# talmolab/VNL-Brax-Imitation

Hardware: NVIDIA B200
Metric: rodent imitation env-steps/s (higher is better)
Workload: dtype f32

## Files before the change

include/vnl_b200.h:

```cpp
#ifndef VNL_B200_H_
#define VNL_B200_H_

#include <stddef.h>
#include <stdint.h>

#ifdef __cplusplus
extern "C" {
#endif

#define VNL_MAGIC_MODEL 0x4d4c4e56u
#define VNL_MAGIC_TASK 0x544c4e56u
#define VNL_BLOB_VERSION 7
#define VNL_TABLE_OFF 64
#define VNL_MAX_FIELDS 96
#define VNL_DATA_OFF (VNL_TABLE_OFF + 2 * VNL_MAX_FIELDS)

enum VnlModelHdr {
  VNL_MH_NQ = 4, VNL_MH_NV, VNL_MH_NU, VNL_MH_NA, VNL_MH_NBODY, VNL_MH_NJNT, VNL_MH_NGEOM,
  VNL_MH_NPAIR,
  VNL_MH_NCON,
  VNL_MH_NLIMIT,
  VNL_MH_NEFC,
  VNL_MH_SOLVER,
  VNL_MH_ITERATIONS, VNL_MH_LS_ITERATIONS,
  VNL_MH_EULERDAMP,
  VNL_MH_NM,
  VNL_MH_NLEVEL,
  VNL_MH_MAXDEPTH,
  VNL_MH_NROOT,
  VNL_MH_NDSLOT,
  VNL_MH_ENV_WARPS,
  VNL_MH_NASLOT,
  VNL_MH_TA,
  VNL_MH_TD,
  VNL_MH_TIMESTEP = 32, VNL_MH_GRAVITY_X, VNL_MH_GRAVITY_Y, VNL_MH_GRAVITY_Z,
  VNL_MH_TOLERANCE, VNL_MH_LS_TOLERANCE, VNL_MH_IMPRATIO, VNL_MH_MEANINERTIA
};

enum VnlModelField {
  VNL_F_BODY_PARENTID = 0,
  VNL_F_BODY_ROOTID,
  VNL_F_BODY_JNTADR,
  VNL_F_BODY_JNTNUM,
  VNL_F_BODY_DOFADR,
  VNL_F_BODY_DOFNUM,
  VNL_F_BODY_POS,
  VNL_F_BODY_QUAT,
  VNL_F_BODY_IPOS,
  VNL_F_BODY_IQUAT,
  VNL_F_BODY_MASS,
  VNL_F_BODY_INERTIA,
  VNL_F_BODY_INVWEIGHT0,
  VNL_F_JNT_TYPE,
  VNL_F_JNT_QPOSADR,
  VNL_F_JNT_DOFADR,
  VNL_F_JNT_BODYID,
  VNL_F_JNT_LIMITED,
  VNL_F_JNT_POS,
  VNL_F_JNT_AXIS,
  VNL_F_JNT_STIFFNESS,
  VNL_F_JNT_RANGE,
  VNL_F_JNT_MARGIN,
  VNL_F_JNT_SOLREF,
  VNL_F_JNT_SOLIMP,
  VNL_F_DOF_BODYID,
// ... 23 lines not shown
  VNL_F_PAIR_GEOM2,
  VNL_F_PAIR_TYPE,
  VNL_F_PAIR_FRICTION,
  VNL_F_PAIR_SOLREF,
  VNL_F_PAIR_SOLIMP,
  VNL_F_PAIR_INCLUDEMARGIN,
  VNL_F_LEVEL_START,
  VNL_F_LEVEL_BODY,
  VNL_F_DOF_MADR,
  VNL_F_M_COL,
  VNL_F_DOF_DEPTH,
  VNL_F_BODY_SUBTREE_END,
  VNL_F_LIMIT_JNT,
  VNL_F_CON_PAIR,
  VNL_F_CON_SIGN,
  VNL_F_GEOMC_BODY,
  VNL_F_GEOMC_POS,
  VNL_F_GEOMC_MAT,
  VNL_F_PLANE_POS,
  VNL_F_PLANE_MAT,
  VNL_F_BODY_IMAT,
  VNL_F_M_ROW,
  VNL_F_BODY_LASTDOF,
  VNL_F_DESC_ADR,
  VNL_F_DESC_ENTRY,
  VNL_F_DOFLEVEL_START,
  VNL_F_DOFLEVEL_DOF,
  VNL_F_DOF_ACTADR,
  VNL_F_DOF_ACTLIST,
  VNL_F_KTAB,
  VNL_F_MODEL_COUNT
};

enum VnlKtab {
  VNL_KT_LVL_START = 0,
  VNL_KT_LVL_BP,
  VNL_KT_PARENT,
  VNL_KT_CHILD_ADR,
  VNL_KT_CHILD_LIST,
  VNL_KT_BODY_DOFADR,
  VNL_KT_BODY_DOFNUM,
  VNL_KT_BODY_TREE,
  VNL_KT_BODY_LASTDOF,
  VNL_KT_SUB_END,
  VNL_KT_ROOTS,
  VNL_KT_MROW,
  VNL_KT_MCOL,
  VNL_KT_DOF_BODY,
  VNL_KT_DPART_ADR,
  VNL_KT_APART_ADR,
  VNL_KT_MADR,
  VNL_KT_EROW,
  VNL_KT_ELVL,
  VNL_KT_DESC_ADR,
  VNL_KT_DESC_SRC,
  VNL_KT_DESC_K,
  VNL_KT_DDOF,
  VNL_KT_DLVL,
  VNL_KT_ANC_START,
  VNL_KT_KITEM,
  VNL_KT_KLVL,
  VNL_KT_PROG_A,
  VNL_KT_PROG_D,
  VNL_KT_COUNT
};
enum VnlKtabScalar { VNL_KS_TA = 0, VNL_KS_TD, VNL_KS_NDSLOT, VNL_KS_NHEIGHT , VNL_KT_NSCALAR };

enum VnlTaskHdr {
  VNL_TH_KIND = 4,
  VNL_TH_CLIP_LEN,
  VNL_TH_REF_LEN,
  VNL_TH_SUB_CLIP_LEN,
  VNL_TH_NTRACK,
  VNL_TH_NJIDX,
  VNL_TH_NAPP,
  VNL_TH_NEE,
  VNL_TH_NFRAMES,
  VNL_TH_OBS_SIZE,
  VNL_TH_TRAJ_SIZE,
  VNL_TH_COM_REF_IDX,
  VNL_TH_TORSO_BODY,
  VNL_TH_REWARD_OLD_STATE,
  VNL_TH_TERM_MEAN,
  VNL_TH_USE_SUBCLIP,
  VNL_TH_OBS_QFRC,
  VNL_TH_COM_FROM_FIELD,
  VNL_TH_ROT_BODY,
  VNL_TH_TRAJ_OLD_FRAME,
  VNL_TH_RACT_ACTION,
  VNL_TH_METRICS_RAW,
  VNL_TH_NCLIPS,
  VNL_TH_HEALTHY_LO = 32, VNL_TH_HEALTHY_HI, VNL_TH_TERM_THRESHOLD, VNL_TH_BODY_ERR_MULT,
  VNL_TH_W_RCOM, VNL_TH_W_RVEL, VNL_TH_W_RTRUNK, VNL_TH_W_RQUAT, VNL_TH_W_RACT, VNL_TH_W_RAPP,
  VNL_TH_DONE_RTRUNK
};

enum VnlTaskField {
  VNL_T_POSITION = 0,
  VNL_T_QUATERNION,
  VNL_T_JOINTS,
  VNL_T_BODY_POSITIONS,
  VNL_T_VELOCITY,
  VNL_T_ANGULAR_VELOCITY,
  VNL_T_JOINTS_VELOCITY,
  VNL_T_BODY_IDXS,
  VNL_T_EE_IDX,
  VNL_T_APP_IDX,
  VNL_T_APP_REF_IDX,
  VNL_T_JOINT_COL,
  VNL_T_CENTER_OF_MASS,
  VNL_TASK_COUNT
};

typedef struct VnlState {
  float* qpos;
  float* qvel;
  float* act;
  float* qacc_warmstart;
  float* xpos;
// ... 109 lines not shown
```

vnl-brax-imitation_b200/csrc/vnl_kernels.cu:

```cuda
#include <cuda_runtime.h>
#include <math.h>
#include <stdint.h>
#include <stdlib.h>


#include "../../include/vnl_blob.h"
#include "vnl_device.cuh"
#include "vnl_kernels.h"

#ifndef VNL_EW
#define VNL_EW 1
#endif
#ifndef VNL_STREAM
#define VNL_STREAM 1
#endif
#ifdef VNL_IEEE
#define VNL_RSQRT(x) (1.0f / sqrtf(x))
#else
#define VNL_RSQRT(x) rsqrtf(x)
#endif
#define VNL_CAT2(a, b) a##b
#define VNL_CAT(a, b) VNL_CAT2(a, b)

namespace vnl {
// ... 21 lines not shown

__device__ __forceinline__ void group_sync(int groups) {
  if (groups <= 1) { __syncthreads(); return; }
  const int W = blockDim.x / kEnvThreads, g = ESLOT * groups / W;
  const int first = (g * W + groups - 1) / groups, last = ((g + 1) * W + groups - 1) / groups;
  asm volatile("bar.sync %0, %1;" ::"r"(9 + g), "r"((last - first) * kEnvThreads) : "memory");
}

__host__ __device__ inline int align4(int x) { return (x + 3) & ~3; }

__host__ __device__ inline void make_layout(const Dims& d, Lay& L) {
  int o = 0;
#define A(name, n) L.name = o; o += align4(n)
  A(qpos, d.nq); A(qvel, d.nv); A(act, d.na); A(ctrl, d.nu); A(warm, d.nv);
  A(cdof, d.nv * 6); A(Mdiag, d.nv); A(Kdiag, d.nv); A(rcom, d.nroot * 3);
  A(qfrc_smooth, d.nv); A(qacc_smooth, d.nv); A(act_dot, d.na); A(ints, 16);
  L.Ms = L.Ks = 0;
  if (!d.stream) { A(Ms, d.nM + 1); A(Ks, d.nM + 1); }
  L.Mn = L.H = L.jr = 0;
  if (d.solver == 2) { A(Mn, d.nM); A(H, d.nv * d.nv); A(jr, 3 * d.nv); }
  const int r0 = o;
  A(xpos, d.nbody * 3); A(xquat, d.nbody * 4); A(cvel, d.nbody * 6);
  const int r0a = o;
  o = r0;
  A(Jaref, d.nefc); A(qacc, d.nv); A(Ma, d.nv); A(grad, d.nv); A(Mgrad, d.nv); A(search, d.nv); A(Mv, d.nv); A(qfrc_con, d.nv);
  if (r0a > o) o = r0a;
  const int r1 = o;
  A(xipos, d.nbody * 3); A(xanchor, d.njnt * 3); A(xaxis, d.njnt * 3);
  const int cacc_n = align4((d.nbody > d.nv ? d.nbody : d.nv) * 6);
  if (o - r1 < cacc_n) o = r1 + cacc_n;
  L.cacc = r1;
  A(t16, d.nbody * kTS);
  int r1end = o;
  o = r1;
  A(part, d.naslot + d.ndslot); A(tmpv, d.nv);
  const int scratch_end = o;
  A(lim_dof, d.nlimit); A(limrow_of_dof, d.nv); A(cbody, d.ncon); A(crel, d.ncon * 3); A(cframe, d.ncon * 6); A(cmu, d.ncon);
  A(efcD, d.nefc); A(Jv, d.nefc > 6 * d.ncon ? d.nefc : 6 * d.ncon);
  if (o > r1end) r1end = o;
  o = r1 + (cacc_n > scratch_end - r1 ? cacc_n : scratch_end - r1);
  A(K, d.nM + 40);
  if (o > r1end) r1end = o;
  o = r1end;
#undef A
  L.total = o;
}

struct __align__(16) Cta {
  Dims d;
  Lay L;
  const uint32_t* mb;
  uint32_t foff[VNL_F_MODEL_COUNT];
  uint32_t o_lvl_start, o_lvl_bp, o_parent, o_child_adr, o_child_list, o_body_dofadr, o_body_dofnum, o_body_tree, o_lastdof, o_sub_end,
      o_roots, o_mrow, o_mcol, o_dof_body, o_dpart_adr, o_apart_adr, o_madr, o_erow, o_elvl, o_desc_adr, o_desc_src, o_desc_k, o_ddof, o_dlvl, o_anc_start, o_kitem, o_klvl, o_prog_a, o_prog_d;
  int TA, TD, ndslot, nheight, lockstep, work_stride;
  float* work;
  long long* prof;
  int prof_env;
  __device__ __forceinline__ const int* fi(int f) const { return (const int*)(mb + foff[f]); }
  __device__ __forceinline__ const float* ff(int f) const { return (const float*)(mb + foff[f]); }
};
constexpr int kCtaFloats = (int)((sizeof(Cta) + 15) / 16 * 4);

#define VNL_SMEM                                                  \
  extern __shared__ __align__(16) float smem[];                    \
  const Cta& c = *reinterpret_cast<const Cta*>(smem);              \
  float* const s = smem + so;
#define TB8(name) (reinterpret_cast<const uint8_t*>(smem) + c.o_##name)
#define TB16(name) reinterpret_cast<const uint16_t*>(reinterpret_cast<const uint8_t*>(smem) + c.o_##name)
#define TB32(name) reinterpret_cast<const uint32_t*>(reinterpret_cast<const uint8_t*>(smem) + c.o_##name)

struct Prof {
  long long* p;
  int t0o;
  __device__ __forceinline__ void mark(int i) const {
    if (p) {
      extern __shared__ __align__(16) float smem[];
      env_sync();
      if (ETID == 0) { long long* t0 = reinterpret_cast<long long*>(smem + t0o); const long long t = clock64(); p[i] += t - *t0; *t0 = t; }
    }
  }
};

#define VNL_LDV(w) (*reinterpret_cast<const float*>(Vb + ((w) & 0x3ffcu)))
#define VNL_LDX(w) (*reinterpret_cast<const float*>(xb + (((w) >> 14) & 0x3fcu)))
#define VNL_FLUSHTO(pt, w) if ((w) < 0xff000000u) { (pt)[(w) >> 24] = acc; acc = 0.0f; }
__device__ __forceinline__ void spmv_section(const uint32_t* __restrict__ prog, int T, const float* __restrict__ V,
                                             const float* __restrict__ x, float* __restrict__ part) {
  const char* Vb = reinterpret_cast<const char*>(V);
  const char* xb = reinterpret_cast<const char*>(x);
  const uint4* pp = reinterpret_cast<const uint4*>(prog) + ETID;
  float acc = 0.0f;
  for (int t = 0; t < T; t += 4, pp += kEnvThreads) {
    const uint4 w = *pp;
    const float v0 = VNL_LDV(w.x), x0 = VNL_LDX(w.x), v1 = VNL_LDV(w.y), x1 = VNL_LDX(w.y);
    const float v2 = VNL_LDV(w.z), x2 = VNL_LDX(w.z), v3 = VNL_LDV(w.w), x3 = VNL_LDX(w.w);
    acc += v0 * x0; VNL_FLUSHTO(part, w.x)
    acc += v1 * x1; VNL_FLUSHTO(part, w.y)
    acc += v2 * x2; VNL_FLUSHTO(part, w.z)
    acc += v3 * x3; VNL_FLUSHTO(part, w.w)
  }
}

__device__ __forceinline__ float* slot_work(const Cta& c) {
  return c.work + (size_t)(blockIdx.x * (blockDim.x / kEnvThreads) + ESLOT) * (size_t)c.work_stride;
}
__device__ __forceinline__ void spill_section(const uint32_t* __restrict__ prog, int T, const float* __restrict__ V, float* __restrict__ g) {
// ... 35 lines not shown
    const float4 va = qa, vb = qb;                                                                \
    const uint4 wa = pp[0], wb = pp[kEnvThreads];                                                 \
    if ((t0) + 24 < T) { qa = __ldcg(gq); qb = __ldcg(gq + kEnvThreads); }                        \
    pp += 2 * kEnvThreads; gq += 2 * kEnvThreads;                                                 \
    const float x0 = VNL_LDX(wa.x), x1 = VNL_LDX(wa.y), x2 = VNL_LDX(wa.z), x3 = VNL_LDX(wa.w);   \
    const float x4 = VNL_LDX(wb.x), x5 = VNL_LDX(wb.y), x6 = VNL_LDX(wb.z), x7 = VNL_LDX(wb.w);   \
    float* const pt = (t0) >= TA ? part + dslot0 : part;                                          \
    acc += va.x * x0; VNL_FLUSHTO(pt, wa.x)                                                       \
    acc += va.y * x1; VNL_FLUSHTO(pt, wa.y)                                                       \
    acc += va.z * x2; VNL_FLUSHTO(pt, wa.z)                                                       \
    acc += va.w * x3; VNL_FLUSHTO(pt, wa.w)                                                       \
    acc += vb.x * x4; VNL_FLUSHTO(pt, wb.x)                                                       \
    acc += vb.y * x5; VNL_FLUSHTO(pt, wb.y)                                                       \
    acc += vb.z * x6; VNL_FLUSHTO(pt, wb.z)                                                       \
    acc += vb.w * x7; VNL_FLUSHTO(pt, wb.w)                                                       \
  }
  for (int t = 0; t < T; t += 24) {
    VNL_BATCH(q0a, q0b, t)
    VNL_BATCH(q1a, q1b, t + 8)
    VNL_BATCH(q2a, q2b, t + 16)
  }
#undef VNL_BATCH
}
#undef VNL_LDV
#undef VNL_LDX
#undef VNL_FLUSHTO

__device__ __noinline__ void mul_m(int so, int xo, int outo) {
  VNL_SMEM
  const int nv = c.d.nv, lane = LANE, tid = ETID;
  const float* const Mdiag = s + c.L.Mdiag;
  const float* const x = s + xo;
  float* const pa = s + c.L.part;
  float* const pd = pa + c.d.naslot;
  if (kStream) {
    spmv_stream_g(TB32(prog_a), c.TA + c.TD, c.TA, slot_work(c), x, pa, c.d.naslot);
  } else {
    spmv_section(TB32(prog_a), c.TA, s + c.L.Ms, x, pa);
    spmv_section(TB32(prog_d), c.TD, s + c.L.Ms, x, pd);
  }
  env_sync();
  const uint8_t* const dpa = TB8(dpart_adr);
  const uint8_t* const apa = TB8(apart_adr);
  float* const out = s + outo;
  for (int i = tid; i < nv; i += kEnvThreads) {
    float acc = Mdiag[i] * x[i];
    for (int q = apa[i]; q < apa[i + 1]; ++q) acc += pa[q];
    for (int q = dpa[i]; q < dpa[i + 1]; ++q) acc += pd[q];
    out[i] = acc;
  }
  env_sync();
}

__device__ __noinline__ void factor(int so, bool damp, bool invert, Prof pf) {
  VNL_SMEM
  const int nv = c.d.nv, nM = c.d.nM, lane = LANE, tid = ETID, maxdepth = c.d.maxdepth;
  float* const F = s + c.L.K;
  const uint16_t* const madr = TB16(madr);
  const uint16_t* const anc_start = TB16(anc_start);
  const uint8_t* const mrow = TB8(mrow);
  const uint8_t* const mcol = TB8(mcol);
  if (damp) {
    const float* damping = c.ff(VNL_F_DOF_DAMPING);
    const float dt = c.d.timestep;
    if (kStream) {
      restore_section(TB32(prog_a), c.TA, F, slot_work(c), 4u * (uint32_t)nM);
    } else {
      for (int e = tid; e < nM; e += kEnvThreads) F[e] = s[c.L.Ms + e];
      env_sync();
    }
    for (int i = tid; i < nv; i += kEnvThreads) F[madr[i]] = s[c.L.Mdiag + i] + dt * damping[i];
    if (tid == 0) F[nM] = 0.0f;
    env_sync();
  }
  for (int i = tid; i < 40; i += kEnvThreads) F[nM + i] = 0.0f;
  env_sync();
  const uint2* const erow = reinterpret_cast<const uint2*>(TB32(erow));
  const uint16_t* const elvl = TB16(elvl);
  const uint16_t* const dsrc = TB16(desc_src);
  {
    int r0 = elvl[0] & 255;
    for (int h = 0; h <= c.nheight; ++h) {
      const int r1 = elvl[h + 1] & 255;
      for (int r = r0 + EWARP; r < r1; r += kEnvWarps) {
        const uint2 w = erow[r];
        const int base = w.x & 0x1fff, n = ((w.x >> 13) & 63) + 1, lg = (w.x >> 19) & 7;
        const int d1 = w.y >> 16;
        float* const Fb = F + base;
        if (n <= 32) {
          const int cc = lane & ((1 << lg) - 1), g = lane >> lg, G = 32 >> lg;
          const bool own = (g == 0) && (cc < n);
          const float* const Fc = F + (cc < n ? cc : 0);
          float acc = own ? Fb[cc] : 0.0f, accb = 0.0f;
          int t = (w.y & 0xffff) + g;
          for (; t < d1; t += 4 * G) {
            const int s0 = dsrc[t], s1 = dsrc[t + G], s2 = dsrc[t + 2 * G], s3 = dsrc[t + 3 * G];
            const float u0 = F[s0], u1 = F[s1], u2 = F[s2], u3 = F[s3];
            const float v0 = Fc[s0], v1 = Fc[s1], v2 = Fc[s2], v3 = Fc[s3];
            acc = fmaf(-u0, v0, acc); accb = fmaf(-u1, v1, accb); acc = fmaf(-u2, v2, acc); accb = fmaf(-u3, v3, accb);
          }
          acc += accb;
          for (int o = 1 << lg; o < 32; o <<= 1) acc += __shfl_xor_sync(FULLMASK, acc, o);
          const float rs = VNL_RSQRT(__shfl_sync(FULLMASK, acc, 0));
          if (own) Fb[cc] = cc == 0 ? rs : acc * rs;
        } else {
          const bool on2 = lane + 32 < n;
          const int c1 = on2 ? lane + 32 : 0;
          float acc = Fb[lane], acc2 = on2 ? Fb[c1] : 0.0f;
          for (int t = w.y & 0xffff; t < d1; ++t) {
            const int s0 = dsrc[t];
            const float u = F[s0];
            acc = fmaf(-u, F[s0 + lane], acc);
            acc2 = fmaf(-u, F[s0 + c1], acc2);
          }
          const float rs = VNL_RSQRT(__shfl_sync(FULLMASK, acc, 0));
          Fb[lane] = lane == 0 ? rs : acc * rs;
          if (on2) Fb[c1] = acc2 * rs;
        }
      }
      r0 = r1;
      env_sync();
    }
  }
  pf.mark(16);
  for (int e = tid; e < nM; e += kEnvThreads) {
    const int b0 = madr[mrow[e]];
    if (e != b0) F[e] = F[e] * F[b0];
  }
  env_sync();
  for (int i = tid; i < nv; i += kEnvThreads) { const int m0 = madr[i]; const float rs = F[m0]; F[m0] = rs * rs; }
  env_sync();
  pf.mark(17);
  if (!invert) return;
  const uint16_t* const kitem = TB16(kitem);
  const uint16_t* const klvl = TB16(klvl);
  int i0 = klvl[1];
  for (int dl = 1; dl <= maxdepth; ++dl) {
    const int i1 = klvl[dl + 1];
    for (int it0 = i0; it0 < i1; it0 += kEnvThreads) {
      const int it = it0 + tid;
      float val = 0.0f;
      float* dst = nullptr;
      if (it < i1) {
        const uint32_t w = kitem[it];
        const int cc = w & 255, base = madr[w >> 8];
        const float* const Fi = F + base;
        const uint16_t* const ai = anc_start + base;
        const float* const Fs = F + cc;
        float a0 = Fi[cc], a1 = 0.0f, a2 = 0.0f, a3 = 0.0f;
        int a = 1;
        for (; a + 3 < cc; a += 4) {
          a0 += Fi[a] * Fs[ai[a] - a];
          a1 += Fi[a + 1] * Fs[ai[a + 1] - a - 1];
          a2 += Fi[a + 2] * Fs[ai[a + 2] - a - 2];
          a3 += Fi[a + 3] * Fs[ai[a + 3] - a - 3];
        }
        for (; a < cc; ++a) a0 += Fi[a] * Fs[ai[a] - a];
        val = -((a0 + a1) + (a2 + a3));
        dst = F + base + cc;
      }
      env_sync();
      if (dst) *dst = val;
      env_sync();
    }
    i0 = i1;
  }
  {
    if (kStream) {
      float* const wk = slot_work(c) + (c.TA + c.TD) * kEnvThreads;
      spill_section(TB32(prog_a), c.TA, F, wk);
      spill_section(TB32(prog_d), c.TD, F, wk + c.TA * kEnvThreads);
    } else {
      for (int e = tid; e <= nM; e += kEnvThreads) s[c.L.Ks + e] = F[e];
    }
    for (int i = tid; i < nv; i += kEnvThreads) s[c.L.Kdiag + i] = F[madr[i]];
    env_sync();
  }
  pf.mark(18);
}

__device__ __noinline__ void solve_m(int so, int xo, int outo) {
  VNL_SMEM
  const int nv = c.d.nv, lane = LANE, tid = ETID;
  const float* const Kdiag = s + c.L.Kdiag;
  const float* const x = s + xo;
  float* const pa = s + c.L.part;
  float* const pd = pa + c.d.naslot;
  float* const tmp = s + c.L.tmpv;
  const uint8_t* const dpa = TB8(dpart_adr);
  const float* const wk = slot_work(c) + (c.TA + c.TD) * kEnvThreads;
  if (kStream) spmv_stream_g(TB32(prog_d), c.TD, 0, wk + c.TA * kEnvThreads, x, pd, 0);
  else spmv_section(TB32(prog_d), c.TD, s + c.L.Ks, x, pd);
  env_sync();
  for (int j = tid; j < nv; j += kEnvThreads) {
    float acc = x[j];
    for (int q = dpa[j]; q < dpa[j + 1]; ++q) acc += pd[q];
    tmp[j] = acc * Kdiag[j];
  }
  env_sync();
  if (kStream) spmv_stream_g(TB32(prog_a), c.TA, c.TA, wk, tmp, pa, 0);
  else spmv_section(TB32(prog_a), c.TA, s + c.L.Ks, tmp, pa);
  env_sync();
  float* const out = s + outo;
  const uint8_t* const apa = TB8(apart_adr);
  for (int i = tid; i < nv; i += kEnvThreads) {
    float acc = tmp[i];
    for (int q = apa[i]; q < apa[i + 1]; ++q) acc += pa[q];
    out[i] = acc;
  }
  env_sync();
}

__device__ __noinline__ void solve_ld(int so, int xo, int outo) {
  VNL_SMEM
  const int nv = c.d.nv, lane = LANE, tid = ETID;
  const float* const F = s + c.L.K;
  const float* const x = s + xo;
  float* const t = s + c.L.tmpv;
  const uint16_t* const madr = TB16(madr);
  const uint8_t* const mcol = TB8(mcol);
  for (int i = tid; i < nv; i += kEnvThreads) t[i] = x[i];
  env_sync();
  {
    const uint2* const erow = reinterpret_cast<const uint2*>(TB32(erow));
    const uint16_t* const elvl = TB16(elvl);
    const uint16_t* const dsrc = TB16(desc_src);
    const uint8_t* const dkk = TB8(desc_k);
    uint32_t lw = elvl[1];
    for (int h = 1; h <= c.nheight; ++h) {
      const uint32_t lw1 = elvl[h + 1];
      const int r0 = lw & 255, r1 = lw1 & 255, lg = lw >> 8;
      const int sl = lane & ((1 << lg) - 1), per = 32 >> lg, W = 1 << lg;
      for (int rs = r0 + EWARP * per; rs < r1; rs += per * kEnvWarps) {
        const int r = rs + (lane >> lg);
        float acc = 0.0f;
        int j = 0;
        if (r < r1) {
          const uint2 w = erow[r];
          j = w.x >> 22;
          const int d1 = w.y >> 16;
          for (int q = (w.y & 0xffff) + sl; q < d1; q += W) acc += F[dsrc[q]] * t[dkk[q]];
        }
        for (int o = W >> 1; o > 0; o >>= 1) acc += __shfl_xor_sync(FULLMASK, acc, o);
        if (r < r1 && sl == 0) t[j] -= acc;
      }
      lw = lw1;
      env_sync();
    }
  }
  for (int i = tid; i < nv; i += kEnvThreads) t[i] *= F[madr[i]];
  env_sync();
  {
    const uint8_t* const ddof = TB8(ddof);
    const uint16_t* const dlvl = TB16(dlvl);
    uint32_t lw = dlvl[0];
    for (int dl = 1; dl <= c.d.maxdepth; ++dl) {
      const uint32_t lw1 = dlvl[dl];
      const int r0 = lw & 255, r1 = lw1 & 255, lg = lw >> 8;
      const int sl = lane & ((1 << lg) - 1), per = 32 >> lg, W = 1 << lg;
      for (int rs = r0 + EWARP * per; rs < r1; rs += per * kEnvWarps) {
        const int r = rs + (lane >> lg);
        float acc = 0.0f;
        int i = 0;
        if (r < r1) {
          i = ddof[r];
          const int base = madr[i];
          for (int a = 1 + sl; a <= dl; a += W) acc += F[base + a] * t[mcol[base + a]];
        }
        for (int o = W >> 1; o > 0; o >>= 1) acc += __shfl_xor_sync(FULLMASK, acc, o);
        if (r < r1 && sl == 0) t[i] -= acc;
      }
      lw = lw1;
      env_sync();
    }
  }
  float* const out = s + outo;
  for (int i = tid; i < nv; i += kEnvThreads) out[i] = t[i];
  env_sync();
}

__device__ __noinline__ void jmul(int so, int xo, int outo) {
  VNL_SMEM
  const int* ints = (const int*)(s + c.L.ints);
  const int nl = ints[0], nc = ints[1], lane = LANE, tid = ETID;
// ... 1304 lines not shown
      const bool over = steps >= p.episode.episode_length;
      const float trunc = over ? 1.0f - done : 0.0f;
      if (over) done = 1.0f;
      if (lane == 0) { p.episode.steps_out[e] = steps; p.episode.truncation_out[e] = trunc; }
    }
    if (lane == 0) {
      p.outputs.reward[e] = nan_to_num(total);
      p.outputs.done[e] = done;
      float* mt = p.outputs.metrics + 7 * (size_t)e;
      mt[0] = r_com; mt[1] = rvl; mt[2] = rtr; mt[3] = rquat; mt[4] = ract; mt[5] = rapp; mt[6] = rtr;
      if (vnl_hdr_i(tb, VNL_TH_METRICS_RAW)) { mt[0] = raw0; mt[1] = raw1; mt[2] = rtrunk; mt[3] = raw3; mt[4] = raw4; mt[5] = raw5; mt[6] = rtrunk; }
    }
    if (p.outputs.stats && lane < 4) p.outputs.stats[4 * e + lane] = stats[lane];
    env_sync();
    if (p.first.qpos && done > 0.0f) {
      const VnlState& f1 = p.first;
      for (int i = tid; i < d.nq; i += kEnvThreads) o.qpos[(size_t)e * d.nq + i] = f1.qpos[(size_t)e * d.nq + i];
      for (int i = tid; i < d.nv; i += kEnvThreads) o.qvel[(size_t)e * d.nv + i] = f1.qvel[(size_t)e * d.nv + i];
      for (int i = tid; i < d.na; i += kEnvThreads) o.act[(size_t)e * d.na + i] = f1.act[(size_t)e * d.na + i];
      for (int i = tid; i < d.nv; i += kEnvThreads) o.qacc_warmstart[(size_t)e * d.nv + i] = f1.qacc_warmstart[(size_t)e * d.nv + i];
      for (int i = tid; i < d.nbody * 3; i += kEnvThreads) o.xpos[(size_t)e * d.nbody * 3 + i] = f1.xpos[(size_t)e * d.nbody * 3 + i];
      for (int i = tid; i < d.nbody * 4; i += kEnvThreads) o.xquat[(size_t)e * d.nbody * 4 + i] = f1.xquat[(size_t)e * d.nbody * 4 + i];
      for (int i = tid; i < d.nv; i += kEnvThreads) o.qfrc_actuator[(size_t)e * d.nv + i] = f1.qfrc_actuator[(size_t)e * d.nv + i];
      if (lane < 3) o.subtree_com[(size_t)e * 3 + lane] = f1.subtree_com[(size_t)e * 3 + lane];
      if (p.first_obs)
        for (int i = tid; i < obs_size; i += kEnvThreads) p.outputs.obs[(size_t)e * obs_size + i] = p.first_obs[(size_t)e * obs_size + i];
    }
  }
  env_sync();
  pf.mark(15);
}

template <int MODE>
__global__ void __launch_bounds__(kMaxEnvs * kEnvThreads, 1) vnl_env_kernel(Params p) {
  extern __shared__ __align__(16) float smem[];
  Cta& c = *reinterpret_cast<Cta*>(smem);
  uint32_t* ktab = reinterpret_cast<uint32_t*>(smem + kCtaFloats);
  const int tid = threadIdx.x, nt = blockDim.x;
  const uint32_t* g_ktab = (const uint32_t*)vnl_field_i(p.model, VNL_F_KTAB);
  for (int i = tid; i < p.dims.ktab_words; i += nt) ktab[i] = g_ktab[i];
  for (int f = tid; f < VNL_F_MODEL_COUNT; f += nt) c.foff[f] = p.model[VNL_TABLE_OFF + 2 * f];
  if (tid == 0) {
    c.d = p.dims;
    make_layout(c.d, c.L);
    c.mb = p.model;
    c.prof = p.prof; c.prof_env = p.prof_env; c.lockstep = p.lockstep;
    c.work = p.work; c.work_stride = p.work_stride;
    const uint32_t kb = (uint32_t)(kCtaFloats * 4);
#define TOFF(name, id) c.o_##name = kb + g_ktab[id]
    TOFF(lvl_start, VNL_KT_LVL_START); TOFF(lvl_bp, VNL_KT_LVL_BP); TOFF(parent, VNL_KT_PARENT); TOFF(child_adr, VNL_KT_CHILD_ADR);
    TOFF(child_list, VNL_KT_CHILD_LIST); TOFF(body_dofadr, VNL_KT_BODY_DOFADR); TOFF(body_dofnum, VNL_KT_BODY_DOFNUM);
    TOFF(body_tree, VNL_KT_BODY_TREE); TOFF(lastdof, VNL_KT_BODY_LASTDOF); TOFF(sub_end, VNL_KT_SUB_END); TOFF(roots, VNL_KT_ROOTS);
    TOFF(mrow, VNL_KT_MROW); TOFF(mcol, VNL_KT_MCOL); TOFF(dof_body, VNL_KT_DOF_BODY); TOFF(dpart_adr, VNL_KT_DPART_ADR); TOFF(apart_adr, VNL_KT_APART_ADR);
    TOFF(madr, VNL_KT_MADR); TOFF(erow, VNL_KT_EROW); TOFF(elvl, VNL_KT_ELVL); TOFF(desc_adr, VNL_KT_DESC_ADR); TOFF(desc_src, VNL_KT_DESC_SRC);
    TOFF(desc_k, VNL_KT_DESC_K); TOFF(ddof, VNL_KT_DDOF); TOFF(dlvl, VNL_KT_DLVL); TOFF(anc_start, VNL_KT_ANC_START); TOFF(kitem, VNL_KT_KITEM);
    TOFF(klvl, VNL_KT_KLVL); TOFF(prog_a, VNL_KT_PROG_A); TOFF(prog_d, VNL_KT_PROG_D);
#undef TOFF
    c.TA = (int)g_ktab[VNL_KT_COUNT + VNL_KS_TA]; c.TD = (int)g_ktab[VNL_KT_COUNT + VNL_KS_TD];
    c.ndslot = (int)g_ktab[VNL_KT_COUNT + VNL_KS_NDSLOT];
    c.nheight = (int)g_ktab[VNL_KT_COUNT + VNL_KS_NHEIGHT];
  }
  __syncthreads();
  const int W = nt / kEnvThreads, warp = tid / kEnvThreads;
  const int so = kCtaFloats + align4(c.d.ktab_words) + warp * c.L.total;
  const int n = MODE == 5 ? p.rs.scratch[0] : p.B;
  const int stride = gridDim.x * W, rounds = (n + stride - 1) / stride;
  for (int r = 0; r < rounds; ++r) {
    const int i = r * stride + warp * gridDim.x + blockIdx.x;
    env_run<MODE>(so, p, MODE == 5 ? (i < n ? p.rs.scratch[1 + i] : 0) : i, i < n);
  }
}

template __global__ void vnl_env_kernel<0>(Params);
template __global__ void vnl_env_kernel<1>(Params);
template __global__ void vnl_env_kernel<2>(Params);
template __global__ void vnl_env_kernel<3>(Params);
template __global__ void vnl_env_kernel<4>(Params);
template __global__ void vnl_env_kernel<5>(Params);

int layout_table(const Dims& d, LayoutEntry* out, int cap) {
  Lay L;
  make_layout(d, L);
  const int nb = d.nbody, nv = d.nv, big = (nb > nv ? nb : nv) * 6;
  const LayoutEntry e[] = {
      {"qpos", L.qpos, d.nq}, {"qvel", L.qvel, nv}, {"act", L.act, d.na}, {"ctrl", L.ctrl, d.nu}, {"warm", L.warm, nv},
      {"cdof", L.cdof, 6 * nv}, {"Mdiag", L.Mdiag, nv}, {"Kdiag", L.Kdiag, nv}, {"rcom", L.rcom, 3 * d.nroot},
      {"qfrc_smooth", L.qfrc_smooth, nv}, {"qacc_smooth", L.qacc_smooth, nv}, {"act_dot", L.act_dot, d.na}, {"ints", L.ints, 16},
      {"Ms", L.Ms, d.stream ? 0 : d.nM + 1}, {"Ks", L.Ks, d.stream ? 0 : d.nM + 1},
      {"Mn", L.Mn, d.solver == 2 ? d.nM : 0}, {"H", L.H, d.solver == 2 ? nv * nv : 0}, {"jr", L.jr, d.solver == 2 ? 3 * nv : 0},
      {"xpos", L.xpos, 3 * nb}, {"xquat", L.xquat, 4 * nb}, {"cvel", L.cvel, 6 * nb},
      {"Jaref", L.Jaref, d.nefc}, {"qacc", L.qacc, nv}, {"Ma", L.Ma, nv}, {"grad", L.grad, nv}, {"Mgrad", L.Mgrad, nv},
      {"search", L.search, nv}, {"Mv", L.Mv, nv}, {"qfrc_con", L.qfrc_con, nv},
      {"xipos", L.xipos, 3 * nb}, {"xanchor", L.xanchor, 3 * d.njnt}, {"xaxis", L.xaxis, 3 * d.njnt}, {"cacc", L.cacc, big},
      {"t16", L.t16, kTS * nb}, {"part", L.part, d.naslot + d.ndslot}, {"tmpv", L.tmpv, nv},
      {"lim_dof", L.lim_dof, d.nlimit}, {"limrow_of_dof", L.limrow_of_dof, nv}, {"cbody", L.cbody, d.ncon}, {"crel", L.crel, 3 * d.ncon},
      {"cframe", L.cframe, 6 * d.ncon}, {"cmu", L.cmu, d.ncon}, {"efcD", L.efcD, d.nefc},
      {"Jv", L.Jv, d.nefc > 6 * d.ncon ? d.nefc : 6 * d.ncon}, {"K", L.K, d.nM + 40}, {"total", L.total, 0}};
  const int n = (int)(sizeof(e) / sizeof(e[0]));
  for (int i = 0; i < n && i < cap; ++i) out[i] = e[i];
  return n;
}

static int max_envs_per_cta(const Dims& d) {
  Lay L;
  make_layout(d, L);
  const int w = (227 * 1024 - (kCtaFloats + align4(d.ktab_words)) * 4) / (L.total * 4);
  return w > kMaxEnvs ? kMaxEnvs : w;
// ... 72 lines not shown
```

vnl-brax-imitation_b200/model_blob.py:

```python
from __future__ import annotations

import os
import re
from typing import Dict, List

import numpy as np

from . import mjcf

_HEADER = os.path.join(os.path.dirname(os.path.abspath(__file__)), "..", "include", "vnl_b200.h")


def _parse_header(path: str):
    txt = open(path).read()
    txt = re.sub(r"/\*.*?\*/", "", txt, flags=re.S)
    consts: Dict[str, int] = {}
    for mm in re.finditer(r"#define\s+(VNL_\w+)\s+(0x[0-9a-fA-F]+u?|\d+)\s*$", txt, flags=re.M):
        consts[mm.group(1)] = int(mm.group(2).rstrip("u"), 0)
    for mm in re.finditer(r"enum\s+\w+\s*\{(.*?)\}", txt, flags=re.S):
        val = -1
        for item in mm.group(1).split(","):
            item = item.strip()
            if not item:
                continue
# ... 150 lines not shown
        lanes = [[] for _ in range(NL)]
        lane_load = [0] * NL
        for slot, terms in sorted(rows, key=lambda r: -len(r[1])):
            l = min(range(NL), key=lambda l: lane_load[l])
            lanes[l].append((slot, terms))
            lane_load[l] += len(terms)
        T = 8 * ((max(1, max(lane_load)) + 7) // 8)
        prog = np.zeros((T, NL), dtype=np.uint32)
        pad = np.uint32((4 * nM_) | (0xFF << 24))
        prog[:, :] = pad
        for l in range(NL):
            t = 0
            for slot, terms in lanes[l]:
                for k, (e, xi) in enumerate(terms):
                    flush = slot if k == len(terms) - 1 else 0xFF
                    prog[t, l] = np.uint32((4 * int(e)) | ((4 * int(xi)) << 14) | (int(flush) << 24))
                    t += 1
        return np.ascontiguousarray(prog.reshape(T // 4, 4, NL).transpose(0, 2, 1)).reshape(-1), T

    CH = 24 if env_warps == 1 else 12
    CHA = 1 << 20 if env_warps == 1 else 12
    rows_a, apart_adr = [], [0]
    for i in range(nv):
        terms = [(madr[i] + a, mcol[madr[i] + a]) for a in range(1, madr[i + 1] - madr[i])]
        for k in range(0, len(terms), CHA):
            rows_a.append((len(rows_a), terms[k:k + CHA]))
        apart_adr.append(len(rows_a))
    if len(rows_a) > 254:
        raise NotImplementedError("too many partial-sum slots for the packed mat-vec program")
    prog_a, TA = pack_program(rows_a) if rows_a else (np.full(8 * NL, np.uint32((4 * nM_) | (0xFF << 24)), dtype=np.uint32), 8)
    naslot = len(rows_a)
    rows_d, dpart_adr = [], [0]
    for j in range(nv):
        terms = [(e, mrow[e]) for e in desc[j]]
        for k in range(0, len(terms), CH):
            rows_d.append((len(rows_d), terms[k:k + CH]))
        dpart_adr.append(len(rows_d))
    if len(rows_d) > 254 or nv > 254:
        raise NotImplementedError("too many partial-sum slots for the packed mat-vec program")
    prog_d, TD = pack_program(rows_d) if rows_d else (np.full(8 * NL, np.uint32((4 * nM_) | (0xFF << 24)), dtype=np.uint32), 8)
    ndslot = len(rows_d)
    lg2c = lambda n: 0 if n <= 1 else min(5, int(np.ceil(np.log2(n))))
    dpar = [int(mcol[madr[i] + 1]) if ddepth[i] > 0 else -1 for i in range(nv)]
    desc_of = [[] for _ in range(nv)]
    height = [0] * nv
    for k in range(nv - 1, -1, -1):
        j, a = dpar[k], 1
        while j >= 0:
            desc_of[j].append((k, a))
            j, a = dpar[j], a + 1
        if dpar[k] >= 0:
            height[dpar[k]] = max(height[dpar[k]], height[k] + 1)
    maxh = max(height) if nv else 0
    erow, elvl, desc_adr, desc_src, desc_k = [], [], [0], [], []
    for j in range(nv):
        for k, a in desc_of[j]:
            desc_src.append(madr[k] + a)
            desc_k.append(k)
        groups = 32 >> lg2c(ddepth[j] + 1) if ddepth[j] + 1 <= 32 else 1
        while desc_of[j] and (len(desc_src) - desc_adr[-1]) % (4 * groups):
            desc_src.append(nM_)
            desc_k.append(0)
        desc_adr.append(len(desc_src))
    if nM_ >= (1 << 13) or len(desc_src) >= (1 << 16):
        raise NotImplementedError("model too large for the packed factorisation schedule")
    for h in range(0, maxh + 1):
        rows = sorted([j for j in range(nv) if height[j] == h], reverse=True)
        elvl.append(len(erow) // 2 | (lg2c(max(len(desc_of[j]) for j in rows)) << 8))
        for j in rows:
            erow += [madr[j] | (int(ddepth[j]) << 13) | (lg2c(ddepth[j] + 1) << 19) | (j << 22), desc_adr[j] | (desc_adr[j + 1] << 16)]
    elvl.append(len(erow) // 2)
    ddof, dlvl = [], []
    for dpt in range(1, maxd + 1):
        dlvl.append(len(ddof) | (lg2c(dpt) << 8))
        ddof += [i for i in range(nv) if ddepth[i] == dpt]
    dlvl.append(len(ddof))
    kitem, klvl = [], [0, 0]
    for dpt in range(1, maxd + 1):
        items = [(c, i) for i in range(nv) if ddepth[i] == dpt for c in range(1, dpt + 1)]
        items.sort(key=lambda t: (-t[0], t[1]))
        kitem += [c | (i << 8) for c, i in items]
        klvl.append(len(kitem))
    u8 = lambda a: np.asarray(a, dtype=np.int64).astype(np.uint8)
    u16 = lambda a: np.asarray(a, dtype=np.int64).astype(np.uint16)
    lastdof_u8 = np.where(lastdof < 0, 0xFF, lastdof)
    kt = [None] * C["VNL_KT_COUNT"]
    kt[C["VNL_KT_LVL_START"]] = u8(level_start)
    kt[C["VNL_KT_LVL_BP"]] = u16([b | (int(parent[b]) << 8) for b in order])
    kt[C["VNL_KT_PARENT"]] = u8(parent)
    kt[C["VNL_KT_CHILD_ADR"]] = u8(child_adr)
    kt[C["VNL_KT_CHILD_LIST"]] = u8([ch for b in range(nb) for ch in children[b]])
    kt[C["VNL_KT_BODY_DOFADR"]] = u8(np.maximum(A["body_dofadr"], 0))
    kt[C["VNL_KT_BODY_DOFNUM"]] = u8(dofnum_flag)
    kt[C["VNL_KT_BODY_TREE"]] = u8(tree)
    kt[C["VNL_KT_BODY_LASTDOF"]] = u8(lastdof_u8)
    kt[C["VNL_KT_SUB_END"]] = u8(sub_end)
    kt[C["VNL_KT_ROOTS"]] = u8(roots)
    kt[C["VNL_KT_MROW"]] = u8(mrow)
    kt[C["VNL_KT_MCOL"]] = u8(mcol)
    kt[C["VNL_KT_DOF_BODY"]] = u8(A["dof_bodyid"])
    kt[C["VNL_KT_DPART_ADR"]] = u8(dpart_adr)
    kt[C["VNL_KT_APART_ADR"]] = u8(apart_adr)
    kt[C["VNL_KT_MADR"]] = u16(madr)
    kt[C["VNL_KT_EROW"]] = np.asarray(erow, dtype=np.int64).astype(np.uint32)
    kt[C["VNL_KT_ELVL"]] = u16(elvl)
    kt[C["VNL_KT_DESC_ADR"]] = u16(desc_adr)
    kt[C["VNL_KT_DESC_SRC"]] = u16(desc_src)
    kt[C["VNL_KT_DESC_K"]] = u8(desc_k)
    kt[C["VNL_KT_DDOF"]] = u8(ddof)
    kt[C["VNL_KT_DLVL"]] = u16(dlvl)
    kt[C["VNL_KT_ANC_START"]] = u16([madr[j] for j in mcol])
    kt[C["VNL_KT_KITEM"]] = u16(kitem)
    kt[C["VNL_KT_KLVL"]] = u16(klvl)
    kt[C["VNL_KT_PROG_A"]] = prog_a
    kt[C["VNL_KT_PROG_D"]] = prog_d
    nkt, nks = C["VNL_KT_COUNT"], C["VNL_KT_NSCALAR"]
    ndir = (nkt + nks + 3) // 4 * 4
    off = 4 * ndir
    dirw = np.zeros(ndir, dtype=np.uint32)
    blobs = []
    for t, a in enumerate(kt):
        raw = a.tobytes()
        raw += b"\0" * ((-len(raw)) % 16)
        dirw[t] = off
        off += len(raw)
        blobs.append(raw)
    assert dirw[C["VNL_KT_PROG_D"]] == dirw[C["VNL_KT_PROG_A"]] + 4 * TA * NL
    dirw[nkt + C["VNL_KS_TA"]] = TA
    dirw[nkt + C["VNL_KS_TD"]] = TD
    dirw[nkt + C["VNL_KS_NDSLOT"]] = ndslot
    dirw[nkt + C["VNL_KS_NHEIGHT"]] = maxh
    ktab = np.frombuffer(dirw.tobytes() + b"".join(blobs), dtype=np.uint32).copy()
    act_of_dof = [[] for _ in range(nv)]
    for u, dadr in enumerate(A["actuator_dofadr"]):
        act_of_dof[int(dadr)].append(u)
    dof_actadr = [0]
    for i in range(nv):
        dof_actadr.append(dof_actadr[-1] + len(act_of_dof[i]))
    return dict(ktab=ktab, TA=TA, TD=TD, env_warps=env_warps, nroot=len(roots), ndslot=ndslot, naslot=naslot, dof_actadr=np.array(dof_actadr),
                dof_actlist=np.array([u for i in range(nv) for u in act_of_dof[i]], dtype=np.int64),
                level_start=np.array(level_start), level_body=np.array(order), dof_madr=np.array(madr),
                m_col=np.array(mcol), dof_depth=np.array(ddepth), body_subtree_end=sub_end,
                limit_jnt=np.array(limit_jnt, dtype=np.int64), con_pair=np.array(con_pair, dtype=np.int64),
                con_sign=np.array(con_sign), geomc_body=A["geom_bodyid"][g2], geomc_pos=A["geom_pos"][g2],
                geomc_mat=geom_mat, plane_pos=A["geom_pos"][g1], plane_mat=plane_mat,
                body_imat=np.array([mjcf.quat_to_mat(q).reshape(9) for q in A["body_iquat"]]),
                m_row=np.array(mrow), body_lastdof=lastdof, desc_adr=np.array(desc_adr),
                desc_entry=np.array(desc_entry, dtype=np.int64), doflevel_start=np.array(dl_start),
                doflevel_dof=np.array(dl_dof, dtype=np.int64),
                nlevel=nlevel, maxdepth=int(max(ddepth)) if ddepth else 0)


_MODEL_FIELDS = [
    ("VNL_F_BODY_PARENTID", "body_parentid", np.int32), ("VNL_F_BODY_ROOTID", "body_rootid", np.int32),
    ("VNL_F_BODY_JNTADR", "body_jntadr", np.int32), ("VNL_F_BODY_JNTNUM", "body_jntnum", np.int32),
    ("VNL_F_BODY_DOFADR", "body_dofadr", np.int32), ("VNL_F_BODY_DOFNUM", "body_dofnum", np.int32),
    ("VNL_F_BODY_POS", "body_pos", np.float32), ("VNL_F_BODY_QUAT", "body_quat", np.float32),
    ("VNL_F_BODY_IPOS", "body_ipos", np.float32), ("VNL_F_BODY_IQUAT", "body_iquat", np.float32),
# ... 166 lines not shown
```

Baseline: 1.144 million.

## Itemize small elimination levels across all env threads in sparse factorization

For height levels of the tree-sparse LDL/Cholesky factorization that have only a few rows and short descendant lists, the blob builder now emits a flat per-element item list. The kernel processes these levels thread-per-element with an unrolled, grouped-summation helper instead of warp-per-row, so idle warps in narrow levels get work. The level table is widened to 32 bits to carry item offsets, and padding is skipped for itemized rows. The cost is an extra sync per itemized batch, more blob complexity, and a different floating-point summation order.

```diff
diff --git a/include/vnl_b200.h b/include/vnl_b200.h
--- a/include/vnl_b200.h
+++ b/include/vnl_b200.h
@@ -10,7 +10,7 @@
 
 #define VNL_MAGIC_MODEL 0x4d4c4e56u
 #define VNL_MAGIC_TASK 0x544c4e56u
-#define VNL_BLOB_VERSION 7
+#define VNL_BLOB_VERSION 8
 #define VNL_TABLE_OFF 64
 #define VNL_MAX_FIELDS 96
 #define VNL_DATA_OFF (VNL_TABLE_OFF + 2 * VNL_MAX_FIELDS)
@@ -140,6 +140,7 @@
   VNL_KT_MADR,
   VNL_KT_EROW,
   VNL_KT_ELVL,
+  VNL_KT_EITEM,
   VNL_KT_DESC_ADR,
   VNL_KT_DESC_SRC,
   VNL_KT_DESC_K,
@@ -153,6 +154,8 @@
   VNL_KT_COUNT
 };
 enum VnlKtabScalar { VNL_KS_TA = 0, VNL_KS_TD, VNL_KS_NDSLOT, VNL_KS_NHEIGHT , VNL_KT_NSCALAR };
+#define VNL_ELIM_ITEM_DESC 8
+#define VNL_ELIM_ITEM_UNROLL 4
 
 enum VnlTaskHdr {
   VNL_TH_KIND = 4,
diff --git a/vnl-brax-imitation_b200/csrc/vnl_kernels.cu b/vnl-brax-imitation_b200/csrc/vnl_kernels.cu
--- a/vnl-brax-imitation_b200/csrc/vnl_kernels.cu
+++ b/vnl-brax-imitation_b200/csrc/vnl_kernels.cu
@@ -97,7 +97,7 @@
   const uint32_t* mb;
   uint32_t foff[VNL_F_MODEL_COUNT];
   uint32_t o_lvl_start, o_lvl_bp, o_parent, o_child_adr, o_child_list, o_body_dofadr, o_body_dofnum, o_body_tree, o_lastdof, o_sub_end,
-      o_roots, o_mrow, o_mcol, o_dof_body, o_dpart_adr, o_apart_adr, o_madr, o_erow, o_elvl, o_desc_adr, o_desc_src, o_desc_k, o_ddof, o_dlvl, o_anc_start, o_kitem, o_klvl, o_prog_a, o_prog_d;
+      o_roots, o_mrow, o_mcol, o_dof_body, o_dpart_adr, o_apart_adr, o_madr, o_erow, o_elvl, o_eitem, o_desc_adr, o_desc_src, o_desc_k, o_ddof, o_dlvl, o_anc_start, o_kitem, o_klvl, o_prog_a, o_prog_d;
   int TA, TD, ndslot, nheight, lockstep, work_stride;
   float* work;
   long long* prof;
@@ -239,6 +239,43 @@
   env_sync();
 }
 
+static_assert(VNL_ELIM_ITEM_DESC == 8, "elim_item sums at most eight lane groups");
+__device__ __forceinline__ float elim_item(const float* F, const uint16_t* ds, int d, int c, int n, float f) {
+  if (n > 32) {
+    for (int q = 0; q < d; ++q) { const int s0 = ds[q]; f = fmaf(-F[s0], F[s0 + c], f); }
+    return f;
+  }
+  const int G = 32 >> (n <= 1 ? 0 : 32 - __clz(n - 1));
+  const int ng = d < G ? (d > 1 ? d : 1) : G;
+  float l0 = 0.0f, l1 = 0.0f, l2 = 0.0f;
+#pragma unroll
+  for (int g = 0; g < VNL_ELIM_ITEM_DESC; ++g) {
+    if (g < ng) {
+      float a = g == 0 ? f : 0.0f, b = 0.0f;
+      for (int q = g, k = 0; q < d; q += G, ++k) {
+        const int s0 = ds[q];
+        if (k & 1) b = fmaf(-F[s0], F[s0 + c], b);
+        else a = fmaf(-F[s0], F[s0 + c], a);
+      }
+      const float p = a + b;
+      if (g == 1 || g == 5) l1 = l0 + p;
+      else if (g == 3) l2 = l1 + (l0 + p);
+      else if (g == 7) l1 = l1 + (l0 + p);
+      else l0 = p;
+    }
+  }
+  switch (ng) {
+    case 1: return l0;
+    case 2: return l1;
+    case 3: return l1 + l0;
+    case 4: return l2;
+    case 5: return l2 + l0;
+    case 6: return l2 + l1;
+    case 7: return l2 + (l1 + l0);
+    default: return l2 + l1;
+  }
+}
+
 __device__ __noinline__ void factor(int so, bool damp, bool invert, Prof pf) {
   VNL_SMEM
   const int nv = c.d.nv, nM = c.d.nM, lane = LANE, tid = ETID, maxdepth = c.d.maxdepth;
@@ -263,13 +300,41 @@
   for (int i = tid; i < 40; i += kEnvThreads) F[nM + i] = 0.0f;
   env_sync();
   const uint2* const erow = reinterpret_cast<const uint2*>(TB32(erow));
-  const uint16_t* const elvl = TB16(elvl);
+  const uint32_t* const elvl = TB32(elvl);
+  const uint16_t* const eitem = TB16(eitem);
+  const uint16_t* const dadr = TB16(desc_adr);
   const uint16_t* const dsrc = TB16(desc_src);
   {
-    int r0 = elvl[0] & 255;
+    constexpr int U = VNL_ELIM_ITEM_UNROLL;
+    uint32_t lw = elvl[0];
     for (int h = 0; h <= c.nheight; ++h) {
-      const int r1 = elvl[h + 1] & 255;
-      for (int r = r0 + EWARP; r < r1; r += kEnvWarps) {
+      const uint32_t lw1 = elvl[h + 1];
+      const int r0 = lw & 255, r1 = (int)(lw1 & 255), i1 = (int)(lw1 >> 16);
+      for (int it0 = (int)(lw >> 16); it0 < i1; it0 += U * kEnvThreads) {
+        int e[U], pv[U], n[U], t0[U], d[U];
+        float acc[U];
+#pragma unroll
+        for (int u = 0; u < U; ++u) {
+          const int it = it0 + u * kEnvThreads + tid;
+          e[u] = it < i1 ? eitem[it] : nM;
+          const int j = it < i1 ? mrow[e[u]] : 0;
+          pv[u] = madr[j];
+          n[u] = madr[j + 1] - pv[u];
+          t0[u] = dadr[j];
+          d[u] = it < i1 ? dadr[j + 1] - t0[u] : 0;
+          acc[u] = F[e[u]];
+        }
+#pragma unroll
+        for (int u = 0; u < U; ++u) {
+          acc[u] = elim_item(F, dsrc + t0[u], d[u], e[u] - pv[u], n[u], acc[u]);
+          if (e[u] == pv[u]) F[e[u]] = VNL_RSQRT(acc[u]);
+        }
+        env_sync();
+#pragma unroll
+        for (int u = 0; u < U; ++u)
+          if (e[u] != pv[u] && e[u] < nM) F[e[u]] = acc[u] * F[pv[u]];
+      }
+      for (int r = i1 > (int)(lw >> 16) ? r1 : r0 + EWARP; r < r1; r += kEnvWarps) {
         const uint2 w = erow[r];
         const int base = w.x & 0x1fff, n = ((w.x >> 13) & 63) + 1, lg = (w.x >> 19) & 7;
         const int d1 = w.y >> 16;
@@ -305,7 +370,7 @@
           if (on2) Fb[c1] = acc2 * rs;
         }
       }
-      r0 = r1;
+      lw = lw1;
       env_sync();
     }
   }
@@ -410,13 +475,13 @@
   env_sync();
   {
     const uint2* const erow = reinterpret_cast<const uint2*>(TB32(erow));
-    const uint16_t* const elvl = TB16(elvl);
+    const uint32_t* const elvl = TB32(elvl);
     const uint16_t* const dsrc = TB16(desc_src);
     const uint8_t* const dkk = TB8(desc_k);
     uint32_t lw = elvl[1];
     for (int h = 1; h <= c.nheight; ++h) {
       const uint32_t lw1 = elvl[h + 1];
-      const int r0 = lw & 255, r1 = lw1 & 255, lg = lw >> 8;
+      const int r0 = lw & 255, r1 = lw1 & 255, lg = (lw >> 8) & 7;
       const int sl = lane & ((1 << lg) - 1), per = 32 >> lg, W = 1 << lg;
       for (int rs = r0 + EWARP * per; rs < r1; rs += per * kEnvWarps) {
         const int r = rs + (lane >> lg);
@@ -1827,7 +1892,7 @@
     TOFF(child_list, VNL_KT_CHILD_LIST); TOFF(body_dofadr, VNL_KT_BODY_DOFADR); TOFF(body_dofnum, VNL_KT_BODY_DOFNUM);
     TOFF(body_tree, VNL_KT_BODY_TREE); TOFF(lastdof, VNL_KT_BODY_LASTDOF); TOFF(sub_end, VNL_KT_SUB_END); TOFF(roots, VNL_KT_ROOTS);
     TOFF(mrow, VNL_KT_MROW); TOFF(mcol, VNL_KT_MCOL); TOFF(dof_body, VNL_KT_DOF_BODY); TOFF(dpart_adr, VNL_KT_DPART_ADR); TOFF(apart_adr, VNL_KT_APART_ADR);
-    TOFF(madr, VNL_KT_MADR); TOFF(erow, VNL_KT_EROW); TOFF(elvl, VNL_KT_ELVL); TOFF(desc_adr, VNL_KT_DESC_ADR); TOFF(desc_src, VNL_KT_DESC_SRC);
+    TOFF(madr, VNL_KT_MADR); TOFF(erow, VNL_KT_EROW); TOFF(elvl, VNL_KT_ELVL); TOFF(eitem, VNL_KT_EITEM); TOFF(desc_adr, VNL_KT_DESC_ADR); TOFF(desc_src, VNL_KT_DESC_SRC);
     TOFF(desc_k, VNL_KT_DESC_K); TOFF(ddof, VNL_KT_DDOF); TOFF(dlvl, VNL_KT_DLVL); TOFF(anc_start, VNL_KT_ANC_START); TOFF(kitem, VNL_KT_KITEM);
     TOFF(klvl, VNL_KT_KLVL); TOFF(prog_a, VNL_KT_PROG_A); TOFF(prog_d, VNL_KT_PROG_D);
 #undef TOFF
diff --git a/vnl-brax-imitation_b200/model_blob.py b/vnl-brax-imitation_b200/model_blob.py
--- a/vnl-brax-imitation_b200/model_blob.py
+++ b/vnl-brax-imitation_b200/model_blob.py
@@ -226,24 +226,28 @@
         if dpar[k] >= 0:
             height[dpar[k]] = max(height[dpar[k]], height[k] + 1)
     maxh = max(height) if nv else 0
-    erow, elvl, desc_adr, desc_src, desc_k = [], [], [0], [], []
+    hrows = [sorted([j for j in range(nv) if height[j] == h], reverse=True) for h in range(maxh + 1)]
+    itemized = [1 < len(rows) <= C["VNL_ELIM_ITEM_UNROLL"] * NL and max(len(desc_of[j]) for j in rows) <= C["VNL_ELIM_ITEM_DESC"]
+                for rows in hrows]
+    erow, elvl, eitem, desc_adr, desc_src, desc_k = [], [], [], [0], [], []
     for j in range(nv):
         for k, a in desc_of[j]:
             desc_src.append(madr[k] + a)
             desc_k.append(k)
         groups = 32 >> lg2c(ddepth[j] + 1) if ddepth[j] + 1 <= 32 else 1
-        while desc_of[j] and (len(desc_src) - desc_adr[-1]) % (4 * groups):
+        while desc_of[j] and not itemized[height[j]] and (len(desc_src) - desc_adr[-1]) % (4 * groups):
             desc_src.append(nM_)
             desc_k.append(0)
         desc_adr.append(len(desc_src))
-    if nM_ >= (1 << 13) or len(desc_src) >= (1 << 16):
-        raise NotImplementedError("model too large for the packed factorisation schedule")
-    for h in range(0, maxh + 1):
-        rows = sorted([j for j in range(nv) if height[j] == h], reverse=True)
-        elvl.append(len(erow) // 2 | (lg2c(max(len(desc_of[j]) for j in rows)) << 8))
+    for h, rows in enumerate(hrows):
+        elvl.append(len(erow) // 2 | (lg2c(max(len(desc_of[j]) for j in rows)) << 8) | (len(eitem) << 16))
         for j in rows:
             erow += [madr[j] | (int(ddepth[j]) << 13) | (lg2c(ddepth[j] + 1) << 19) | (j << 22), desc_adr[j] | (desc_adr[j + 1] << 16)]
-    elvl.append(len(erow) // 2)
+        if itemized[h]:
+            eitem += [madr[j] for j in rows] + [madr[j] + c for j in rows for c in range(1, int(ddepth[j]) + 1)]
+    elvl.append(len(erow) // 2 | (len(eitem) << 16))
+    if nM_ >= (1 << 13) or len(desc_src) >= (1 << 16) or len(eitem) >= (1 << 16):
+        raise NotImplementedError("model too large for the packed factorisation schedule")
     ddof, dlvl = [], []
     for dpt in range(1, maxd + 1):
         dlvl.append(len(ddof) | (lg2c(dpt) << 8))
@@ -277,7 +281,8 @@
     kt[C["VNL_KT_APART_ADR"]] = u8(apart_adr)
     kt[C["VNL_KT_MADR"]] = u16(madr)
     kt[C["VNL_KT_EROW"]] = np.asarray(erow, dtype=np.int64).astype(np.uint32)
-    kt[C["VNL_KT_ELVL"]] = u16(elvl)
+    kt[C["VNL_KT_ELVL"]] = np.asarray(elvl, dtype=np.int64).astype(np.uint32)
+    kt[C["VNL_KT_EITEM"]] = u16(eitem)
     kt[C["VNL_KT_DESC_ADR"]] = u16(desc_adr)
     kt[C["VNL_KT_DESC_SRC"]] = u16(desc_src)
     kt[C["VNL_KT_DESC_K"]] = u8(desc_k)
```

Result: slower. 1.029 million (median of 6 runs) (-10.1%).
